# google-deepmind/dm_control

Hardware: AMD Instinct MI355X
Metric: env-steps/s (whole node) at batch 4096; max rel qpos error vs CPU (higher is better)
Workload: dtype f32

## Files before the change

### dm_control_amd/csrc/step_core.h

```cpp
#pragma once
#include <math.h>
#include <stdint.h>
#ifdef DMC_HOST_EMU
#include <stdio.h>
#include <stdlib.h>
#include <string.h>
#endif

#include "../../include/dmc_model_layout.h"
#include "step_layout.h"

#ifdef DMC_HOST_EMU
#define DMC_DEV inline
#define DMC_FN inline
#define DMC_LDS
#define DMC_GLB
#define DMC_WSYNC() ((void)++dmc_emu_wsync_count)
static long long dmc_emu_wsync_count = 0;
#else
#define DMC_DEV __device__ __forceinline__
#define DMC_FN __device__ __attribute__((noinline, not_tail_called))
#define DMC_LDS __attribute__((address_space(3)))
#define DMC_GLB __attribute__((address_space(1)))
#define DMC_WSYNC()                                             \
// ... 2625 lines not shown
      const int a0 = MI(level_adr)[lev], cnt = MI(level_adr)[lev + 1] - a0;
      for (int idx = lane; idx < cnt*6; idx += LPE) {
        const int b = MI(level_body)[a0 + idx/6], comp = idx % 6;
        const int c0 = MI(child_adr)[b], c1 = MI(child_adr)[b + 1];
        if (c1 > c0) {
          T v = S(cfrc)[6*b + comp];
          for (int c = c0; c < c1; c++) v += S(cfrc)[6*MI(child_list)[c] + comp];
          S(cfrc)[6*b + comp] = v;
        }
      }
      DMC_WSYNC();
    }
    FOR_LANES(i, nv) S(qfrc_bias)[i] = dot_n(S(cdof) + 6*i, S(cfrc) + 6*MI(dof_bodyid)[i], 6);
    DMC_WSYNC();
  }

  DMC_DEV void subtree_linvel_sensors() {
    for (int k = 0; k < L.d.nstv; k++) {
      const int sidx = MI(stv_sensor)[k], root = MI(sensor_objid)[sidx];
      T mom[3] = {0, 0, 0};
      FOR_LANES(i, L.d.nbody) {
        const unsigned m = (unsigned)(root < 32 ? MI(body_anc_lo)[i] : MI(body_anc_hi)[i]);
        if (!((m >> (root & 31)) & 1u)) continue;
        const T* rc = S(subtree_com) + 3*MI(body_rootid)[i];
        T dif[3] = {S(xipos)[3*i] - rc[0], S(xipos)[3*i + 1] - rc[1], S(xipos)[3*i + 2] - rc[2]}, tmp[3];
        cross3(tmp, dif, S(cvel) + 6*i);
        for (int c = 0; c < 3; c++) mom[c] += MR(body_mass)[i] * (S(cvel)[6*i + 3 + c] - tmp[c]);
      }
      const T inv = 1 / t_max((T)DMC_MINVAL, MR(body_subtreemass)[root]);
      for (int c = 0; c < 3; c++) { const T v = group_sum<LPE>(mom[c]) * inv; if (lane == 0) S(sensordata)[MI(sensor_adr)[sidx] + c] = v; }
    }
  }
  DMC_DEV void object_velocity(int body, const T* pos, const T* mat, T* res) {
    const T* rc = S(subtree_com) + 3*MI(body_rootid)[body];
    T dif[3] = {pos[0] - rc[0], pos[1] - rc[1], pos[2] - rc[2]}, tmp[3];
    const T* cv = S(cvel) + 6*body;
    cross3(tmp, dif, cv);
    T lin[3] = {cv[3] - tmp[0], cv[4] - tmp[1], cv[5] - tmp[2]};
    mul_matT_vec3(res, mat, cv); mul_matT_vec3(res + 3, mat, lin);
  }
  DMC_DEV void contact_force_local(int c, T* f6) {
    for (int k = 0; k < 6; k++) f6[k] = 0;
    const int r0 = SI(con_efc)[c];
    if (r0 < 0) return;
    const int dim = con_dim(c);
    const T* f = S(efc_force) + r0;
    if (dim == 1) { f6[0] = f[0]; return; }
    if (L.d.elliptic) { for (int k = 0; k < dim; k++) f6[k] = f[k]; return; }
    for (int k = 0; k < 2*(dim - 1); k++) f6[0] += f[k];
    for (int k = 1; k < dim; k++) f6[k] = (f[2*(k - 1)] - f[2*(k - 1) + 1]) * MR(prm_friction)[3*con_prm(c) + (k < 3 ? 0 : (k == 3 ? 1 : 2))];
  }
  DMC_DEV void rne_post_constraint() {
    const int nb = L.d.nbody, ncon = SI(imisc)[IM_NCON];
    FOR_LANES(b, nb) {
      T acc[6] = {0, 0, 0, 0, 0, 0};
      if (b > 0) for (int c = 0; c < ncon; c++) {
        if (SI(con_efc)[c] < 0) continue;
        const int b1 = con_b1(c), b2 = con_b2(c);
        if (b1 != b && b2 != b) continue;
        T lf[6], gf[3], gt[3], dif[3], t[3];
        contact_force_local(c, lf);
        mul_matT_vec3(gf, conF() + 9*c, lf); mul_matT_vec3(gt, conF() + 9*c, lf + 3);
        const T* rc = S(subtree_com) + 3*MI(body_rootid)[b];
        for (int k = 0; k < 3; k++) dif[k] = S(con_pos)[3*c + k] - rc[k];
        cross3(t, dif, gf);
        if (b1 == b) for (int k = 0; k < 3; k++) { acc[k] += -(gt[k] + t[k]); acc[3 + k] += -gf[k]; }
        if (b2 == b) for (int k = 0; k < 3; k++) { acc[k] += (gt[k] + t[k]); acc[3 + k] += gf[k]; }
      }
      if (b > 0 && o.xfrc) {
        T xf[6], dif[3], t[3]; load_xfrc(b, xf);
        const T* rc = S(subtree_com) + 3*MI(body_rootid)[b];
        for (int k = 0; k < 3; k++) dif[k] = S(xipos)[3*b + k] - rc[k];
        cross3(t, dif, xf);
        for (int k = 0; k < 3; k++) { acc[k] += xf[3 + k] + t[k]; acc[3 + k] += xf[k]; }
      }
      for (int k = 0; k < 6; k++) S(cfrc_ext)[6*b + k] = acc[k];
    }
    if (lane == 0) {
      T* ca = S(cacc);
      ca[0] = ca[1] = ca[2] = 0; ca[3] = ca[4] = ca[5] = 0;
      if (!(o.disableflags & DMC_DSBL_GRAVITY)) { ca[3] = -o.gravity[0]; ca[4] = -o.gravity[1]; ca[5] = -o.gravity[2]; }
      for (int k = 0; k < 6; k++) S(cfrc)[k] = 0;
    }
    DMC_WSYNC();
    for (int lev = 0; lev < L.d.nlevel; lev++) {
      const int a0 = MI(level_adr)[lev], a1 = MI(level_adr)[lev + 1];
      for (int kk = a0 + lane; kk < a1; kk += LPE) {
        const int i = MI(level_body)[kk], bda = MI(body_dofadr)[i];
        T csum[6], tmp[6], tmp1[6], tmp2[6];
        for (int a = 0; a < 6; a++) csum[a] = S(cacc)[6*MI(body_parentid)[i] + a];
        for (int k = 0; k < MI(body_dofnum)[i]; k++) for (int a = 0; a < 6; a++)
          csum[a] += SG(cdof_dot)[6*(bda + k) + a]*S(qvel)[bda + k] + S(cdof)[6*(bda + k) + a]*S(qacc)[bda + k];
        for (int a = 0; a < 6; a++) S(cacc)[6*i + a] = csum[a];
        mul_inert_vec(tmp, SG(cinert) + 10*i, csum);
        mul_inert_vec(tmp1, SG(cinert) + 10*i, S(cvel) + 6*i);
        cross_force(tmp2, S(cvel) + 6*i, tmp1);
        for (int a = 0; a < 6; a++) S(cfrc)[6*i + a] = tmp[a] + tmp2[a] - S(cfrc_ext)[6*i + a];
      }
      DMC_WSYNC();
    }
    for (int lev = L.d.nlevel - 2; lev >= 0; lev--) {
      const int a0 = MI(level_adr)[lev], cnt = MI(level_adr)[lev + 1] - a0;
      for (int idx = lane; idx < cnt*6; idx += LPE) {
        const int b = MI(level_body)[a0 + idx/6], comp = idx % 6;
        const int c0 = MI(child_adr)[b], c1 = MI(child_adr)[b + 1];
        if (c1 > c0) {
// ... 1936 lines not shown
          if (lane == 0) S(efc_force)[i] = f;
          if (delta != 0) { const T* Ap = ns_A() + i*cap; for (int b = lane; b < nefc; b += LPE) S(ns_res)[b] += Ap[b]*delta; }
          DMC_WSYNC();
          improvement -= change;
        } else if (dim == 3) improvement -= pgs_cone_block<3>(i);
        else if (dim == 4) improvement -= pgs_cone_block<4>(i);
        else improvement -= pgs_cone_block<6>(i);
        i += dim;
      }
      improvement *= scale;
      iter++;
      if (improvement < o.tolerance) break;
    }
    constraint_force_to_joint(nefc);
    DMC_WSYNC();
    chol_solve(S(sv_Mgrad), M_factor(), S(qfrc_constraint), nv, true);
    FOR_LANES(i, nv) { const T a = S(qacc_smooth)[i] + S(sv_Mgrad)[i]; S(qacc)[i] = a; S(qacc_warmstart)[i] = a; }
    if (lane == 0) SI(imisc)[IM_ITER] = iter;
    DMC_WSYNC();
  }
  DMC_DEV void fwd_constraint() {
    const int nv = L.d.nv, nefc = SI(imisc)[IM_NEFC];
    if (!nefc) {
      FOR_LANES(i, nv) { const T a = S(qacc_smooth)[i]; S(qacc)[i] = a; S(qacc_warmstart)[i] = a; S(qfrc_constraint)[i] = 0; }
      if (lane == 0) SI(imisc)[IM_ITER] = 0;
      DMC_WSYNC();
      return;
    }
    if (L.d.pgs) {
      pgs_solve(nefc);
      if (L.d.nslip) { if (o.noslip_iterations > 0) noslip(nefc); }
      return;
    }
    int changed = 1;
    T cc = 0, gauss = 0;
    bool evaluated = false;
    if (!(o.disableflags & DMC_DSBL_WARMSTART)) {
      jar_from(S(qacc_smooth), nefc);
      DMC_WSYNC();
      const T cs = constraint_update(nefc);
      FOR_LANES(i, nv) S(qacc)[i] = S(qacc_warmstart)[i];
      DMC_WSYNC();
      jar_from(S(qacc), nefc);
      mul_M(S(sv_Ma), S(qacc));
      DMC_WSYNC();
      for (int i = lane; i < nefc; i += LPE) SI(efc_active)[i] = -1;
      cc = constraint_update(nefc, &changed);
      gauss = gauss_cost();
      if (cc + gauss > cs) FOR_LANES(i, nv) S(qacc)[i] = S(qacc_smooth)[i];
      else evaluated = true;
    } else FOR_LANES(i, nv) S(qacc)[i] = S(qacc_smooth)[i];
    DMC_WSYNC();
    int iter;
    if (L.d.island && (o.islands < 0 ? (sizeof(T) == 8 || L.d.cg) : o.islands != 0) && !(o.disableflags & DMC_DSBL_ISLAND) && solve_islands(nefc, &iter)) constraint_force_to_joint(nefc);
    else {
      iter = primal_solve(nefc, evaluated, cc, gauss, changed);
    }
    FOR_LANES(i, nv) S(qacc_warmstart)[i] = S(qacc)[i];
    if (lane == 0) SI(imisc)[IM_ITER] = iter;
    DMC_WSYNC();
    DMC_PROF(PROF_SOL_UPD);
    if (L.d.nslip) { if (o.noslip_iterations > 0) noslip(nefc); }
    DMC_PROF(PROF_NOSLIP);
  }
#if !defined(DMC_HOST_EMU) && !defined(DMC_NO_NEWTON_REGS)
#ifndef DMC_NEWTON_REGS_F64_NV
#define DMC_NEWTON_REGS_F64_NV 0
#endif
  static constexpr bool kNewtonRegs = LS::kNV > 0 && LS::kNV <= 16 && LS::kNV <= LPE && LPE >= 16
                                      && (sizeof(T) == 4 || LS::kNV <= DMC_NEWTON_REGS_F64_NV);
#else
  static constexpr bool kNewtonRegs = false;
#endif
#ifndef DMC_EPS_IMP
#define DMC_EPS_IMP 1
#endif
  static constexpr int kNewtonRows = 16;
#ifndef DMC_HOST_EMU
  template <int N> DMC_DEV T nr_dot(const T (&m)[N], T v) const {
#pragma clang fp contract(off)
    T s = 0;
#pragma unroll
    for (int j = 0; j < N; j++) { const T t = m[j] * bcast_rows<LPE, N>(v, j); s = s + t; }
    return s;
  }
  DMC_DEV T nr_jtf(const T (&Jc)[kNewtonRows], T force, int nefc) const {
#pragma clang fp contract(off)
    T f = 0;
#pragma unroll
    for (int r = 0; r < kNewtonRows; r += 4) if (r < nefc) {
      T fr[4];
#pragma unroll
      for (int u = 0; u < 4; u++) fr[u] = bcast_rows<LPE, kNewtonRows>(force, r + u);
#pragma unroll
      for (int u = 0; u < 4; u++) {
        if constexpr (sizeof(T) == 4) { if (u < 2) { const T t = Jc[r + u]*fr[u]; f = f + t; } else f = __builtin_fmaf(Jc[r + u], fr[u], f); }
        else f = fr[u] != 0 ? f + Jc[r + u]*fr[u] : f;
      }
    }
    return f;
  }
  template <int N> DMC_DEV void nr_factor(const T (&M)[N], const T (&Jc)[kNewtonRows], T wD, int nefc, T (&row)[N], T (&col)[N], T& dinv) const {
    const bool own = lane < N;
    T a[N];
#pragma unroll
    for (int j = 0; j < N; j++) { a[j] = M[j]; col[j] = 0; }
#pragma unroll
    for (int r = 0; r < kNewtonRows; r += 4) if (r < nefc) {
      T c[4];
#pragma unroll
      for (int u = 0; u < 4; u++) c[u] = bcast_rows<LPE, kNewtonRows>(wD, r + u)*Jc[r + u];
#pragma unroll
      for (int u = 0; u < 4; u++) {
#pragma unroll
        for (int j = 0; j < N; j++) a[j] += c[u] * bcast_rows<LPE, N>(Jc[r + u], j);
      }
    }
    dinv = 0;
#pragma unroll
    for (int k = 0; k < N; k++) {
      T akk = bcast_rows<LPE, N>(a[k], k);
      if (akk < (T)DMC_MINVAL) akk = (T)DMC_MINVAL;
      const T inv = t_rsqrt(akk);
      const T lik = a[k] * inv;
#pragma unroll
      for (int j = k + 1; j < N; j++) {
        const T ljk = bcast_rows<LPE, N>(lik, j);
        a[j] = nmsub<true>(a[j], lik, ljk);
        col[j] = lane == k ? ljk : col[j];
      }
      row[k] = (own && k < lane) ? lik : (T)0;
      dinv = lane == k ? inv : dinv;
    }
  }
  template <int N> DMC_DEV T nr_solve(const T (&row)[N], const T (&col)[N], T dinv, T b) const {
    T sreg = lane < N ? b : (T)0;
#pragma unroll
    for (int k = 0; k < N; k++) { const T xk = bcast_rows<LPE, N>(sreg*dinv, k); sreg = nmsub<true>(sreg, row[k], xk); }
    sreg = sreg*dinv;
#pragma unroll
    for (int k = N - 1; k >= 0; k--) { const T xk = bcast_rows<LPE, N>(sreg*dinv, k); sreg = nmsub<true>(sreg, col[k], xk); }
    return sreg*dinv;
  }
  DMC_DEV T nr_update(bool rown, T jar, T D, T& force, int& act, int* changed) const {
    T cost = 0;
    int ch = 0;
    if (rown) {
      const int a = jar < 0;
      const T dj = D*jar;
      force = a ? -dj : (T)0;
      if (sizeof(T) == 4) cost += a ? (T)0.5*dj*jar : (T)0; else if (a) cost += (T)0.5*D*jar*jar;
      ch |= act != a; act = a;
    }
    cost = group_sum<LPE>(cost);
    *changed = group_max<LPE>(ch);
    return cost;
  }
  template <int N>
  DMC_DEV int primal_solve_regs(int nefc, bool evaluated, T cc, T gauss, int changed) {
    const bool own = lane < N, rown = lane < nefc;
    const int i = own ? lane : 0, rl = rown ? lane : 0;
    const T scale = 1 / (o.meaninertia * (T)(N > 1 ? N : 1));
    constexpr bool keep = sizeof(T) == 4;
    T M[N], Jr[N], Jc[kNewtonRows], row[N], col[N], dinv = 0;
    auto load_M = [&]() __attribute__((always_inline)) {
      asm volatile("" ::: "memory");
#pragma unroll
      for (int j = 0; j < N; j++) M[j] = S(qM)[i*N + j];
    };
    auto load_Jr = [&]() __attribute__((always_inline)) {
#pragma unroll
      for (int j = 0; j < N; j++) Jr[j] = S(efc_Jd)[rl*N + j];
    };
    load_M(); load_Jr();
#pragma unroll
    for (int r = 0; r < kNewtonRows; r++) {
      const int t = r & ~3, rr = r < nefc ? r : (t < nefc ? t : 0);
      Jc[r] = S(efc_Jd)[rr*N + i];
    }
    T qacc = S(qacc)[i];
    const T qas = S(qacc_smooth)[i], qfs = S(qfrc_smooth)[i];
    const T D_ = S(efc_D)[rl], aref_ = S(efc_aref)[rl], Ma_ = S(sv_Ma)[i], jar_ = S(efc_jar)[rl], force_ = S(efc_force)[rl];
    const int act_ = SI(efc_active)[rl];
    const T D = rown ? D_ : (T)0;
    T Ma, jar, force = 0;
    int act;
    auto gauss_cost_regs = [&]() __attribute__((always_inline)) {
      T g = 0;
      if (own) g += (Ma - qfs) * (qacc - qas);
      return (T)0.5 * group_sum<LPE>(g);
    };
    if (!evaluated) {
      Ma = nr_dot<N>(M, qacc);
      const T ja = nr_dot<N>(Jr, qacc) - aref_;
      jar = rown ? ja : (T)0;
      changed = 1;
      act = -1;
      cc = nr_update(rown, jar, D, force, act, &changed);
      gauss = gauss_cost_regs();
    } else { Ma = Ma_; jar = rown ? jar_ : (T)0; force = rown ? force_ : (T)0; act = act_; }
    T cost = cc + gauss;
    DMC_PROF(PROF_SOL_INIT);
    T fc, grad, Mgrad;
    auto gradient_regs = [&](int refactor) __attribute__((always_inline)) {
      fc = nr_jtf(Jc, force, nefc);
      grad = Ma - qfs - fc;
      DMC_PROF(PROF_SOL_GRAD);
      if (refactor) {
        if constexpr (!keep) load_M();
        nr_factor<N>(M, Jc, (rown && act == EFC_ST_QUADRATIC) ? D : (T)0, nefc, row, col, dinv);
        DMC_PROF(PROF_FACTOR);
      }
      Mgrad = nr_solve<N>(row, col, dinv, grad);
      DMC_PROF(PROF_SOLVE);
    };
    gradient_regs(1);
    T search = -Mgrad;
    DMC_PROF(PROF_SOL_GRAD);
    int iter = 0;
    const bool anch = anchored();
    while (iter < o.iterations) {
      if (iter == DMC_PRIO_ITER) __builtin_amdgcn_s_setprio(2);
      T lscost = 0;
      DMC_TSUB(3, iter == 0, 4);
      if constexpr (!keep) { load_M(); load_Jr(); }
      const T Mv = nr_dot<N>(M, search);
      const T jv_ = nr_dot<N>(Jr, search);
      const T jv = rown ? jv_ : (T)0;
      T a1 = 0, a2 = 0, a3 = 0, a4 = 0;
      if (own) {
        const T sr = search;
        if (anch) a1 += sr*grad;
        else { a1 += sr*Ma; a2 += qfs*sr; }
        a3 += sr*Mv; a4 += sr*sr;
      }
      LSPre pre;
      pre.a1 = a1; pre.a2 = a2; pre.a3 = a3; pre.a4 = a4; pre.jar = jar; pre.jv = jv; pre.D = D;
      const T alpha = primal_search<true>(nefc, gauss, scale, &lscost, pre);
      DMC_PROF(PROF_SOL_LS);
      DMC_TSUB(3, iter == 0, 5);
      if (alpha == 0) break;
      if constexpr (sizeof(T) == 4) {
        qacc = __builtin_fmaf(alpha, search, qacc); Ma = __builtin_fmaf(alpha, Mv, Ma);
        jar = __builtin_fmaf(alpha, jv, jar);
      } else { qacc += alpha*search; Ma += alpha*Mv; jar += alpha*jv; }
      const T oldcost = cost;
      cc = nr_update(rown, jar, D, force, act, &changed);
      gauss = gauss_cost_regs();
      cost = cc + gauss;
      DMC_PROF(PROF_SOL_UPD);
      DMC_TSUB(3, iter == 0, 6);
      gradient_regs(changed);
      DMC_PROF(PROF_SOL_GRAD);
      DMC_TSUB(3, iter == 0, 7);
      T g2 = 0, ma2 = 0;
      search = -Mgrad;
      if (own) { g2 += grad*grad; ma2 += Ma*Ma; }
      g2 = group_sum<LPE>(g2); ma2 = group_sum<LPE>(ma2);
      const T improvement = ls_relative<T>() ? -scale*lscost : scale*(oldcost - cost), gradient = scale*t_sqrt(g2);
      iter++;
      const T ulp = sizeof(T) == 4 ? (T)1.1920929e-7 : (T)2.220446049250313e-16;
      const T tol_imp = ls_relative<T>() ? o.tolerance : t_max(o.tolerance, (T)DMC_EPS_IMP*ulp*scale*t_abs(cost));
      const bool exact_step = sizeof(T) == 4 && !changed && t_abs(alpha - 1) < (T)1e-3;
      const T tol_grad = t_max(o.tolerance, (exact_step ? 64 : 8)*ulp*scale*t_sqrt(ma2));
      if (improvement < tol_imp || gradient < tol_grad) break;
    }
    __builtin_amdgcn_s_setprio(0);
    if (own) { S(qacc)[lane] = qacc; S(qfrc_constraint)[lane] = fc; }
    if (rown) { S(efc_force)[lane] = force; S(efc_jar)[lane] = jar; SI(efc_active)[lane] = act; }
    DMC_WSYNC();
    return iter;
  }
#endif
  DMC_DEV int primal_solve(int nefc, bool evaluated, T cc, T gauss, int changed) {
#ifndef DMC_HOST_EMU
    if constexpr (kNewtonRegs) {
      if (L.d.jfull && !L.d.msparse && !L.d.elliptic && !L.d.cg && !L.d.nslip && !general_rows() && nefc <= kNewtonRows)
        return primal_solve_regs<LS::kNV>(nefc, evaluated, cc, gauss, changed);
    }
#endif
    const int nv = L.d.nv;
    const T scale = 1 / (o.meaninertia * (T)(nv > 1 ? nv : 1));
    if (!evaluated) {
      mul_M(S(sv_Ma), S(qacc));
      jar_from(S(qacc), nefc);
      DMC_WSYNC();
      changed = 1;
      for (int i = lane; i < nefc; i += LPE) SI(efc_active)[i] = -1;
      cc = constraint_update(nefc, &changed);
      gauss = gauss_cost();
    }
    T cost = cc + gauss;
#ifdef DMC_HOST_EMU
    hsplit = !L.d.cg && h_split(nefc);
    emu_split_solves() += hsplit ? 1 : 0;
#else
    hsplit = false;
    if constexpr (kSplit) hsplit = !L.d.cg && h_split(nefc);
#endif
#ifdef DMC_HOST_EMU
    if (getenv("DMC_EMU_TRACE_SPLIT")) fprintf(stderr, "h_split %d (treemax %d, ncon %d)\n", (int)hsplit, L.d.treemax, SI(imisc)[IM_NCON]);
#endif
    DMC_PROF(PROF_SOL_INIT);
    newton_gradient(nefc, 1);
    FOR_LANES(i, nv) S(sv_search)[i] = -S(sv_Mgrad)[i];
    DMC_WSYNC();
    DMC_PROF(PROF_SOL_GRAD);
    int iter = 0, stall = 0;
    T gbest = (T)DMC_MAXVAL;
#ifndef DMC_STALL_ITERS
#define DMC_STALL_ITERS 6
#endif
    while (iter < o.iterations) {
#ifndef DMC_HOST_EMU
      if (iter == DMC_PRIO_ITER) __builtin_amdgcn_s_setprio(2);
#endif
      T lscost;
      DMC_TSUB(3, iter == 0, 4);
      const T alpha = primal_search(nefc, gauss, scale, &lscost);
      DMC_PROF(PROF_SOL_LS);
      DMC_TSUB(3, iter == 0, 5);
#ifdef DMC_HOST_EMU
      if (getenv("DMC_EMU_TRACE_LS")) fprintf(stderr, "    ls returned alpha %.9e lscost %.6e\n", (double)alpha, (double)lscost);
#endif
      if (alpha == 0) break;
      FOR_LANES(i, nv) { S(qacc)[i] += alpha*S(sv_search)[i]; S(sv_Ma)[i] += alpha*S(sv_Mv)[i]; }
// ... 117 lines not shown
      const u64 C = isl_comp(t);
      if (!C || ctz64(C) != t || !(C & rowtrees)) continue;
      FOR_LANES(i, nv) S(qacc)[i] = ((C >> dof_root(i)) & 1) ? S(qacc_warmstart)[i] : S(qacc_smooth)[i];
      for (int r = lane; r < nefc; r += LPE) if (!(row_trees(r) & C)) S(efc_D)[r] *= eps;
      DMC_WSYNC();
      const int it = primal_solve(nefc, false, 0, 0, 1);
      FOR_LANES(i, nv) if ((C >> dof_root(i)) & 1) S(qacc_warmstart)[i] = S(qacc)[i];
      for (int r = lane; r < nefc; r += LPE) if (!(row_trees(r) & C)) S(efc_D)[r] *= 1 / eps;
      DMC_WSYNC();
      if (it > itmax) itmax = it;
    }
    FOR_LANES(i, nv) S(qacc)[i] = ((covered >> dof_root(i)) & 1) ? S(qacc_warmstart)[i] : S(qacc_smooth)[i];
    DMC_WSYNC();
    jar_from(S(qacc), nefc);
    DMC_WSYNC();
    constraint_update(nefc);
    DMC_WSYNC();
    *iter_out = itmax;
    return true;
  }

  DMC_DEV void euler_state() {
    const int nv = L.d.nv;
    const T dt = o.timestep;
    const T* qacc = S(qacc);
    const bool implicitfast = kFeat && o.integrator == DMC_INT_IMPLICITFAST;
    if (implicitfast) {
      FOR_LANES(i, nv) {
        T dd = (o.disableflags & DMC_DSBL_DAMPER) ? (T)0 : MR(dof_damping)[i];
        if (!(o.disableflags & DMC_DSBL_ACTUATION)) for (int a = 0; a < L.d.nu; a++) {
          const int fl = MI(act_flags)[a];
          if ((fl & ACTF_TENDON) || MI(act_dof)[a] != i) continue;
          if (fl & ACTF_FORCELIMITED) { const T f = S(actuator_force)[a]; if (f <= MRC(act_forcerange)[2*a] || f >= MRC(act_forcerange)[2*a + 1]) continue; }
          T bv = (fl & ACTF_BIAS_AFFINE) ? MRC(act_biasprm)[3*a + 2] : (T)0;
          const T gv = (fl & ACTF_GAIN_AFFINE) ? MRC(act_gainprm)[3*a + 2] : (T)0;
          if (gv != 0) bv += gv * ((L.d.na && (fl & ACTF_DYN_ANY)) ? S(act)[MI(act_adr)[a]] : S(ctrl)[a]);
          const T gear = MRC(act_gear)[a];
          dd -= gear*gear*bv;
        }
        S(sv_search)[i] = dd;
      }
      DMC_WSYNC();
    }
    if (L.d.na) FOR_LANES(i, L.d.nu) {
      const int fl = MI(act_flags)[i];
      if (fl & ACTF_DYN_ANY) {
        const int k = MI(act_adr)[i];
        if (fl & ACTF_DYN_FILTEREXACT) { const T tau = t_max((T)DMC_MINVAL, MR(act_dynprm)[i]); S(act)[k] += S(act_dot)[k] * tau * (1 - t_exp(-dt/tau)); }
        else S(act)[k] += dt*S(act_dot)[k];
        if (fl & ACTF_ACTLIMITED) S(act)[k] = t_max(MRC(act_actrange)[2*i], t_min(MRC(act_actrange)[2*i + 1], S(act)[k]));
      }
    }
    if (implicitfast || (o.any_damping && !(o.disableflags & (DMC_DSBL_EULERDAMP | DMC_DSBL_DAMPER)))) {
      FOR_LANES(i, nv) S(sv_grad)[i] = S(qfrc_smooth)[i] + S(qfrc_constraint)[i];
      DMC_WSYNC();
      factor_M(true, implicitfast ? S(sv_search) : MR(dof_damping));
      chol_solve(S(sv_Mgrad), S(qLH), S(sv_grad), nv, true);
      qacc = S(sv_Mgrad);
    }
    FOR_LANES(i, nv) S(qvel)[i] += dt*qacc[i];
    DMC_WSYNC();
    FOR_LANES(j, L.d.njnt) {
      const int qa = MI(jnt_qposadr)[j], da = MI(jnt_dofadr)[j], t = MI(jnt_type)[j];
      if (t == DMC_JNT_FREE) {
        for (int k = 0; k < 3; k++) S(qpos)[qa + k] += dt*S(qvel)[da + k];
        T q[4], w[3];
        for (int k = 0; k < 4; k++) q[k] = S(qpos)[qa + 3 + k];
        for (int k = 0; k < 3; k++) w[k] = S(qvel)[da + 3 + k];
        quat_integrate(q, w, dt);
        for (int k = 0; k < 4; k++) S(qpos)[qa + 3 + k] = q[k];
      } else if (t == DMC_JNT_BALL) {
        T q[4], w[3];
        for (int k = 0; k < 4; k++) q[k] = S(qpos)[qa + k];
        for (int k = 0; k < 3; k++) w[k] = S(qvel)[da + k];
        quat_integrate(q, w, dt);
        for (int k = 0; k < 4; k++) S(qpos)[qa + k] = q[k];
      } else S(qpos)[qa] += dt*S(qvel)[da];
    }
    DMC_WSYNC();
  }
  DMC_DEV void euler() { euler_state(); time_ += o.timestep_d; }

  DMC_DEV void integrate_pos_from(const T* q0, const T* vel, T h) {
    FOR_LANES(j, L.d.njnt) {
      const int qa = MI(jnt_qposadr)[j], da = MI(jnt_dofadr)[j], t = MI(jnt_type)[j];
      if (t == DMC_JNT_FREE || t == DMC_JNT_BALL) {
        int qo = qa, dofo = da;
        if (t == DMC_JNT_FREE) { for (int k = 0; k < 3; k++) S(qpos)[qa + k] = q0[qa + k] + h*vel[da + k]; qo += 3; dofo += 3; }
        T q[4], w[3];
        for (int k = 0; k < 4; k++) q[k] = q0[qo + k];
        for (int k = 0; k < 3; k++) w[k] = vel[dofo + k];
        quat_integrate(q, w, h);
        for (int k = 0; k < 4; k++) S(qpos)[qo + k] = q[k];
      } else S(qpos)[qa] = q0[qa] + h*vel[da];
    }
  }
  DMC_DEV void rk4_stage(int stage) {
    const int nv = L.d.nv;
    const T h = o.timestep;
    const T Bw = (stage == 0 || stage == 3) ? (T)(1.0/6) : (T)(1.0/3);
    if (stage == 0) {
      FOR_LANES(i, L.d.nq) S(rk_q0)[i] = S(qpos)[i];
      FOR_LANES(i, nv) { S(rk_v0)[i] = S(qvel)[i]; S(rk_dq)[i] = Bw*S(qvel)[i]; S(rk_dv)[i] = Bw*S(qacc)[i]; }
    } else FOR_LANES(i, nv) { S(rk_dq)[i] += Bw*S(qvel)[i]; S(rk_dv)[i] += Bw*S(qacc)[i]; }
    DMC_WSYNC();
    if (stage < 3) {
      const T a = stage == 2 ? (T)1 : (T)0.5;
      FOR_LANES(i, nv) { S(sv_grad)[i] = a*S(qvel)[i]; S(sv_Mgrad)[i] = a*S(qacc)[i]; }
      DMC_WSYNC();
      integrate_pos_from(S(rk_q0), S(sv_grad), h);
      FOR_LANES(i, nv) S(qvel)[i] = S(rk_v0)[i] + h*S(sv_Mgrad)[i];
      DMC_WSYNC();
    }
  }
  DMC_DEV void rk4_finish() {
    const T h = o.timestep;
    FOR_LANES(i, L.d.nv) S(qvel)[i] = S(rk_v0)[i] + h*S(rk_dv)[i];
    integrate_pos_from(S(rk_q0), S(rk_dq), h);
    time_ += o.timestep_d;
    DMC_WSYNC();
  }

  DMC_DEV void reset_state() {
    FOR_LANES(i, L.d.nq) S(qpos)[i] = MR(qpos0)[i];
    FOR_LANES(i, L.d.nv) { S(qvel)[i] = 0; S(qacc_warmstart)[i] = 0; S(qfrc_applied)[i] = 0; }
    FOR_LANES(i, L.d.nu) S(ctrl)[i] = 0;
    if (L.d.na) FOR_LANES(i, L.d.na) { S(act)[i] = 0; S(act_dot)[i] = 0; }
    time_ = 0;
    DMC_WSYNC();
  }
  DMC_DEV bool check_pos_vel() {
    int badp = 0, badv = 0;
    FOR_LANES(i, L.d.nq) if (t_bad(S(qpos)[i])) badp = 1;
    badp = group_max<LPE>(badp);
    if (badp) { if (lane == 0) SI(imisc)[IM_WARN + DMC_WARN_BADQPOS]++; if (!(o.disableflags & DMC_DSBL_AUTORESET)) { DMC_WSYNC(); reset_state(); } }
    FOR_LANES(i, L.d.nv) if (t_bad(S(qvel)[i])) badv = 1;
    badv = group_max<LPE>(badv);
    if (badv) { if (lane == 0) SI(imisc)[IM_WARN + DMC_WARN_BADQVEL]++; if (!(o.disableflags & DMC_DSBL_AUTORESET)) { DMC_WSYNC(); reset_state(); } }
    return (badp || badv) && !(o.disableflags & DMC_DSBL_AUTORESET);
  }
  DMC_DEV bool bad_acc() {
    int bad = 0;
    FOR_LANES(i, L.d.nv) if (t_bad(S(qacc)[i])) bad = 1;
    return group_max<LPE>(bad) != 0;
  }

  DMC_DEV void stage_posvel(bool partial, int outmask, bool skipsensor, bool havekin = false) {
    if (!havekin) { kinematics(); DMC_PROF(PROF_KIN); DMC_TSUB(1, partial, 4); com_pos(); DMC_PROF(PROF_COM); DMC_TSUB(1, partial, 5); }
    if (!partial) { crb_mass_matrix(); DMC_PROF(PROF_CRB); DMC_TSUB(2, true, 4); }
    if (!partial || (outmask & (OUT_CONTACT | OUT_CONTACT_IDS))) { collision(); DMC_PROF(PROF_COLL); DMC_TSUB(2, !partial, 5); }
    if (!partial) { make_constraint(); DMC_PROF(PROF_CONSTR); DMC_TSUB(2, true, 6); }
    if (!skipsensor) sensors(DMC_STAGE_POS);
    DMC_PROF(PROF_SENS);
    DMC_TSUB(1, partial, 6);
    if (!havekin) { com_vel(); DMC_PROF(PROF_COMVEL); DMC_TSUB(1, partial, 7); }
    if (!partial) { passive_and_rne(); DMC_PROF(PROF_RNE); DMC_TSUB(2, true, 7); }
    if (!skipsensor) sensors(DMC_STAGE_VEL);
    DMC_PROF(PROF_SENS);
  }
  DMC_DEV void stage_acc(bool disable_actuation, bool skipsensor) {
    fwd_actuation(disable_actuation); DMC_PROF(PROF_ACT); fwd_acceleration(); DMC_PROF(PROF_ACC); fwd_constraint();
    DMC_PROF(PROF_X8);
    if (!skipsensor) sensors_acc();
    DMC_PROF(PROF_SENS);
  }
  DMC_DEV void sub_stamp(int row) {
#if defined(DMC_TRACE_SUB) && !defined(DMC_HOST_EMU)
    const StepIO<T>* iop = (const StepIO<T>*)((const unsigned char*)&o + (sizeof(StepOpts<T>) + 15) / 16 * 16);
    if (iop->trace && (threadIdx.x & 63) == 0) {
      const int epw = 64 / LPE, nitems = (iop->B + epw - 1) / epw;
      iop->trace[((size_t)(iop->trace_slot & 7) * 8 + row) * nitems + SI(imisc)[IM_ENV] / epw] = (int)(wall_clock64() & 0x7fffffffll);
    }
#else
    (void)row;
#endif
  }
  DMC_DEV void trace_stamp(const StepIO<T>& io, int env, int row) {
#if !defined(DMC_HOST_EMU) && !defined(DMC_TRACE_SUB)
    if (io.trace && (threadIdx.x & 63) == 0) {
      const int epw = 64 / LPE, nitems = (io.B + epw - 1) / epw;
      io.trace[((size_t)(io.trace_slot & 7) * 8 + row) * nitems + env / epw] = (int)(wall_clock64() & 0x7fffffffll);
    }
#else
    (void)io; (void)env; (void)row;
#endif
  }
  DMC_DEV void prof_begin() {
#if defined(DMC_PROFILE) && !defined(DMC_HOST_EMU)
    if (lane == 0) { for (int k = 0; k < 33; k++) SI(prof)[k] = 0; SI(prof)[33] = (int)__builtin_readcyclecounter(); }
#endif
  }
  DMC_DEV void prof_end(const StepIO<T>& io, int env) {
#if defined(DMC_PROFILE) && !defined(DMC_HOST_EMU)
    if (io.prof && lane == 0) for (int k = 0; k < 32; k++) io.prof[(size_t)k*io.B + env] += SI(prof)[k];
#else
    (void)io; (void)env;
#endif
  }
#ifndef DMC_HOST_EMU
  DMC_DEV void call_posvel(bool partial, int outmask, bool skipsensor, bool havekin = false) {
    StageFns<T, LPE, LS>::posvel(ls, (const DMC_LDS StepOpts<T>*)&o, (DMC_LDS int*)mi, (DMC_LDS T*)mr, gc, (DMC_LDS T*)s,
                                 (DMC_LDS int*)si, lane, (partial ? 1 : 0) | (skipsensor ? 2 : 0) | (havekin ? 4 : 0), outmask);
  }
  DMC_DEV void call_acc(bool disable_actuation, bool skipsensor) {
    StageFns<T, LPE, LS>::acc(ls, (const DMC_LDS StepOpts<T>*)&o, (DMC_LDS int*)mi, (DMC_LDS T*)mr, gc, (DMC_LDS T*)s,
                              (DMC_LDS int*)si, lane, (disable_actuation ? 1 : 0) | (skipsensor ? 2 : 0));
  }
  DMC_DEV void call_euler() {
    StageFns<T, LPE, LS>::euler(ls, (const DMC_LDS StepOpts<T>*)&o, (DMC_LDS int*)mi, (DMC_LDS T*)mr, gc, (DMC_LDS T*)s,
                                (DMC_LDS int*)si, lane);
    time_ += o.timestep_d;
  }
#else
  DMC_DEV void call_posvel(bool partial, int outmask, bool skipsensor, bool havekin = false) { stage_posvel(partial, outmask, skipsensor, havekin); }
  DMC_DEV void call_acc(bool disable_actuation, bool skipsensor) { stage_acc(disable_actuation, skipsensor); }
  DMC_DEV void call_euler() { euler(); }
#endif
  DMC_DEV void load_ctrl_seq(const StepIO<T>& io, int env, int t) {
    env = late(env);
    const int B = io.B, nu = L.d.nu;
    DMC_WSYNC();
    FOR_LANES(i, nu) S(ctrl)[i] = io.ctrl_seq[((size_t)t*nu + i)*B + env];
    DMC_WSYNC();
  }
  DMC_DEV void store_seq(const StepIO<T>& io, int env, int t) {
    env = late(env);
    const int B = io.B;
    if (io.qpos_seq) FOR_LANES(i, L.d.nq) io.qpos_seq[((size_t)t*L.d.nq + i)*B + env] = S(qpos)[i];
    if (io.qvel_seq) FOR_LANES(i, L.d.nv) io.qvel_seq[((size_t)t*L.d.nv + i)*B + env] = S(qvel)[i];
    if (io.sensor_seq) FOR_LANES(i, L.d.nsensordata) io.sensor_seq[((size_t)t*L.d.nsensordata + i)*B + env] = S(sensordata)[i];
  }
  DMC_DEV void run_split(const StepIO<T>& io, int env, int mode, int outmask, const Entry& en) {
    const bool stash = io.stash_r != nullptr;
    bool have = false;
    if (lane == 0) set_epoch(en.epoch);
    DMC_WSYNC();
    if (mode == 5 && stash) have = load_stash(io, env);
    load_state(io, env, have, en);
    if (mode == 4) {
      check_pos_vel();
      call_posvel(false, outmask, false);
      store_outputs(io, env, outmask);
      if (stash) store_stash(io, env, true);
      store_state(io, env);
      return;
    }
    int retried = 0;
    for (;;) {
      if (!have || retried) call_posvel(false, outmask, true);
      call_acc(false, false);
      if (!retried && bad_acc()) {
        if (lane == 0) SI(imisc)[IM_WARN + DMC_WARN_BADQACC]++;
        if (!(o.disableflags & DMC_DSBL_AUTORESET)) { DMC_WSYNC(); reset_state(); retried = 1; continue; }
      }
      break;
    }
    store_outputs(io, env, outmask & (OUT_SENSOR | OUT_QACC | OUT_ACTUATOR | OUT_QFRC | OUT_CONTACT));
    call_euler();
    if (stash) store_stash(io, env, false);
    store_state(io, env);
  }
  DMC_DEV TaskLds<T> task_lds() const {
    TaskLds<T> v;
    v.qpos = S(qpos); v.qvel = S(qvel); v.ctrl = S(ctrl); v.act = S(act); v.sensordata = S(sensordata); v.xpos = S(xpos);
    v.xmat = S(xmat); v.xipos = S(xipos); v.subtree_com = S(subtree_com); v.geom_xpos = S(geom_xpos); v.cvel = S(cvel);
    return v;
  }
  DMC_DEV void probe_store(const StepIO<T>& io, int env, int first, int count) {
    if constexpr (!kFeat) return;
    env = late(env);
    T* p = io.probe;
    if (!p) return;
    const int cap = io.probe_cap, g = io.probe_geom;
    for (int t = first; t < first + count && t < cap; t++) FOR_LANES(k, 3) p[((size_t)t*3 + k)*io.B + env] = S(geom_xpos)[3*g + k];
  }
  DMC_DEV void run(const StepIO<T>& io, int env, int nstep, int legacy, int mode, int outmask, int nsub) {
    Entry en; EntryRegs er;
    entry_issue(L, o, io, env, lane, mode, legacy, &en, &er);
    entry_commit(L, io, env, lane, &en, er, s);
    run(io, env, nstep, legacy, mode, outmask, nsub, en);
  }
  DMC_DEV void run(const StepIO<T>& io, int env, int nstep, int legacy, int mode, int outmask, int nsub, const Entry& en,
                   int piece = 0, int npieces = 1) {
    const int launch_mode = mode;
    if (lane == 0) set_epoch(en.epoch);
    if (io.env_mode) {
      const int em = en.em;
      if (em == 2) return;
      if (em == 1 && (mode == 0 || mode >= 4)) mode = 2;
    }
    if constexpr (!kSlices) { piece = 0; npieces = 1; }
    if (mode != 0 && piece != npieces - 1) return;
    if (mode != 0) { piece = 0; npieces = 1; }
    if (mode >= 4) { run_split(io, env, mode, outmask, en); return; }
    prof_begin();
    const bool stash = io.stash_r != nullptr;
    bool have = false;
    if (stash && mode == 0 && legacy && o.integrator != DMC_INT_RK4) have = load_stash(io, env);
    load_state(io, env, have, en, kSlices && piece > 0);
    bool havekin = false;
    if (piece == 0 && io.kstash && mode == 0 && launch_mode == 0 && legacy && !have && o.integrator != DMC_INT_RK4) {
      if (!en.fast) havekin = load_kstash(io, env);
      else if (en.kvalid) { havekin = true; DMC_WSYNC(); kstash_env_geoms(); }
    }
    DMC_PROF(PROF_LOAD);
    const bool stepping = mode == 0 || mode == 3;
    const int ntotal = mode == 3 ? nstep*nsub : nstep;
    const int npass = !stepping ? 1 : ntotal + ((legacy || mode == 3) ? 1 : 0);
    const bool fwd_after = kFeat && legacy == 2 && mode == 0;
    const bool last_piece = piece == npieces - 1;
    const int it_lo = npieces > 1 ? (int)((long long)piece * ntotal / npieces) : 0;
    const int it_hi = (npieces > 1 && !last_piece) ? (int)((long long)(piece + 1) * ntotal / npieces) : npass;
    for (int it = it_lo; it < it_hi; it++) {
      const bool trailing = stepping && it == ntotal;
      const bool partial = trailing && !(stash && mode == 0) && !fwd_after;
      if (mode == 3 && !trailing && it % nsub == 0 && io.ctrl_seq) load_ctrl_seq(io, env, it / nsub);
      if (stepping) { if (check_pos_vel()) { have = false; havekin = false; } }
      const int nstage = (stepping && !trailing && o.integrator == DMC_INT_RK4) ? 4 : 1;
      const bool sens_pv = !stepping || it == npass - 1 || (mode == 3 && it % nsub == 0);
      const bool sens_acc = !stepping || (it == ntotal - 1 && !fwd_after) || (trailing && fwd_after) || (mode == 3 && (it + 1) % nsub == 0);
      int stage = 0, retried = 0;
      while (stage < nstage) {
        if (!(have && it == 0 && !retried)) call_posvel(partial, outmask, stage > 0 || !sens_pv, havekin && it == 0 && !retried && !trailing);
        if (it == 0 && stage == 0) trace_stamp(io, env, 4); else if (trailing) trace_stamp(io, env, 7);
        if (mode == 3 && stage == 0 && it > 0 && it % nsub == 0) store_seq(io, env, it / nsub - 1);
        if (mode == 0 && stage == 0 && it >= 1) probe_store(io, env, it - 1, 1);
        if (trailing && !fwd_after) break;
        call_acc(mode == 2, stage > 0 || !sens_acc);
        if (trailing) break;
        if (it == 0 && stage == 0) trace_stamp(io, env, 5);
        if (stage == 0 && stepping && !retried && bad_acc()) {
          if (lane == 0) SI(imisc)[IM_WARN + DMC_WARN_BADQACC]++;
          if (!(o.disableflags & DMC_DSBL_AUTORESET)) { DMC_WSYNC(); reset_state(); retried = 1; continue; }
        }
        if (stage == 0 && stepping && it == ntotal - 1) { dump_debug(io, env); if (mode == 0 && !legacy) store_outputs(io, env, outmask); }
        if (nstage > 1) rk4_stage(stage);
        stage++;
      }
      if (!stepping || trailing) break;
      if (nstage > 1) rk4_finish(); else call_euler();
      if (it == 0) trace_stamp(io, env, 6);
      DMC_PROF(PROF_EULER);
    }
    if constexpr (kSlices) if (!last_piece) { store_handoff(io, env); DMC_PROF(PROF_STORE); prof_end(io, env); return; }
    if (!stepping) dump_debug(io, env);
    if (!stepping && launch_mode == 0) probe_store(io, env, 0, nstep);
    if (!stepping || legacy || mode == 3) { DMC_PROF(PROF_TRAIL); store_outputs(io, env, outmask); }
    if (stash) store_stash(io, env, mode == 0 && legacy && !fwd_after);
    if (io.kstash && mode == 0 && legacy && o.integrator != DMC_INT_RK4) store_kstash(io, env);
    store_state(io, env);
    DMC_PROF(PROF_STORE);
    prof_end(io, env);
  }
#undef MI
#undef MR
#undef GC
#undef S
#undef SG
#undef SI
#undef FOR_LANES
};


#ifndef DMC_HOST_EMU
template <typename T, int LPE, typename LS>
struct StageFns {
  typedef StepCore<T, LPE, LS> Core;
  static DMC_FN void posvel(LS ls, const DMC_LDS StepOpts<T>* o, DMC_LDS int* mi, DMC_LDS T* mr, const int* gc, DMC_LDS T* s,
                            DMC_LDS int* si, int lane, int flags, int outmask) {
    Core c(ls, *(const StepOpts<T>*)o, (const int*)mi, (const T*)mr, gc, (T*)s, (int*)si, lane);
    c.stage_posvel(flags & 1, outmask, flags & 2, flags & 4);
  }
  static DMC_FN void acc(LS ls, const DMC_LDS StepOpts<T>* o, DMC_LDS int* mi, DMC_LDS T* mr, const int* gc, DMC_LDS T* s,
                         DMC_LDS int* si, int lane, int flags) {
    Core c(ls, *(const StepOpts<T>*)o, (const int*)mi, (const T*)mr, gc, (T*)s, (int*)si, lane);
    c.stage_acc(flags & 1, flags & 2);
  }
  static DMC_FN void ns_build(LS ls, const DMC_LDS StepOpts<T>* o, DMC_LDS int* mi, DMC_LDS T* mr, const int* gc, DMC_LDS T* s,
                              DMC_LDS int* si, int lane, int nf) {
    if constexpr (LS::kNV > 0 && LS::kNV <= 32 && LPE == 64) {
      Core c(ls, *(const StepOpts<T>*)o, (const int*)mi, (const T*)mr, gc, (T*)s, (int*)si, lane);
      c.template noslip_build_A_lanes<LS::kNV>((const DMC_LDS T*)c.M_factor(), nf, c.row_map());
    }
  }
  static DMC_FN void euler(LS ls, const DMC_LDS StepOpts<T>* o, DMC_LDS int* mi, DMC_LDS T* mr, const int* gc, DMC_LDS T* s,
                           DMC_LDS int* si, int lane) {
    Core c(ls, *(const StepOpts<T>*)o, (const int*)mi, (const T*)mr, gc, (T*)s, (int*)si, lane);
    c.euler_state();
  }
};
#endif

}
```

Baseline: 76.55 million.

## Fuse smooth acceleration, constraint solve and damped Euler solve into register path

For small dense models with few constraint rows, stage_acc now runs a register-resident path that computes qfrc_smooth/qacc_smooth from the existing M factor, does the warmstart comparison and Newton solve in registers, and skips fwd_acceleration/fwd_constraint. When a plain Euler step with damping follows, it also factors M+dt*damping in registers and solves for the next qacc, and flags euler() to skip its own factor and solve. This removes LDS round trips and wave syncs between stages. It adds register pressure and a shared flag in misc, and the result may differ numerically from the LDS path.

```diff
diff --git a/dm_control_amd/csrc/step_core.h b/dm_control_amd/csrc/step_core.h
--- a/dm_control_amd/csrc/step_core.h
+++ b/dm_control_amd/csrc/step_core.h
@@ -2701,6 +2701,7 @@
   }
   DMC_DEV void rne_post_constraint() {
     const int nb = L.d.nbody, ncon = SI(imisc)[IM_NCON];
+    if constexpr (kAccRegs) { if (lane == 0) S(misc)[kMiscEulerSolved] = 0; }
     FOR_LANES(b, nb) {
       T acc[6] = {0, 0, 0, 0, 0, 0};
       if (b > 0) for (int c = 0; c < ncon; c++) {
@@ -4743,7 +4744,7 @@
     } else FOR_LANES(i, nv) S(qacc)[i] = S(qacc_smooth)[i];
     DMC_WSYNC();
     int iter;
-    if (L.d.island && (o.islands < 0 ? (sizeof(T) == 8 || L.d.cg) : o.islands != 0) && !(o.disableflags & DMC_DSBL_ISLAND) && solve_islands(nefc, &iter)) constraint_force_to_joint(nefc);
+    if (islands_on() && solve_islands(nefc, &iter)) constraint_force_to_joint(nefc);
     else {
       iter = primal_solve(nefc, evaluated, cc, gauss, changed);
     }
@@ -4767,6 +4768,12 @@
 #define DMC_EPS_IMP 1
 #endif
   static constexpr int kNewtonRows = 16;
+#if !defined(DMC_NO_ACC_REGS)
+  static constexpr bool kAccRegs = kNewtonRegs;
+#else
+  static constexpr bool kAccRegs = false;
+#endif
+  static constexpr int kMiscEulerSolved = 2;
 #ifndef DMC_HOST_EMU
   template <int N> DMC_DEV T nr_dot(const T (&m)[N], T v) const {
 #pragma clang fp contract(off)
@@ -4844,11 +4851,39 @@
       ch |= act != a; act = a;
     }
     cost = group_sum<LPE>(cost);
-    *changed = group_max<LPE>(ch);
+    if (changed) *changed = group_max<LPE>(ch);
     return cost;
   }
-  template <int N>
-  DMC_DEV int primal_solve_regs(int nefc, bool evaluated, T cc, T gauss, int changed) {
+  template <int N> DMC_DEV void nr_factor_diag(const T (&M)[N], T dt, T d, T (&row)[N], T (&col)[N], T& dinv) const {
+#pragma clang fp contract(off)
+    const bool own = lane < N;
+    const T dv = dt*d;
+    T a[N];
+#pragma unroll
+    for (int j = 0; j < N; j++) {
+      T v = M[j] + dv;
+      if constexpr (sizeof(T) == 4) { if (j == N - 1 && (N & 1)) v = __builtin_fmaf(dt, d, M[j]); }
+      a[j] = (j == lane) ? v : M[j]; col[j] = 0;
+    }
+    dinv = 0;
+#pragma unroll
+    for (int k = 0; k < N; k++) {
+      T akk = bcast_rows<LPE, N>(a[k], k);
+      if (akk < (T)DMC_MINVAL) akk = (T)DMC_MINVAL;
+      const T inv = t_rsqrt(akk);
+      const T lik = a[k] * inv;
+#pragma unroll
+      for (int j = k + 1; j < N; j++) {
+        const T ljk = bcast_rows<LPE, N>(lik, j);
+        a[j] = nmsub<true>(a[j], lik, ljk);
+        col[j] = lane == k ? ljk : col[j];
+      }
+      row[k] = (own && k < lane) ? lik : (T)0;
+      dinv = lane == k ? inv : dinv;
+    }
+  }
+  template <int N, bool ACC = false>
+  DMC_DEV int primal_solve_regs(int nefc, bool evaluated, T cc, T gauss, int changed, bool euler_next = false) {
     const bool own = lane < N, rown = lane < nefc;
     const int i = own ? lane : 0, rl = rown ? lane : 0;
     const T scale = 1 / (o.meaninertia * (T)(N > 1 ? N : 1));
@@ -4869,10 +4904,29 @@
       const int t = r & ~3, rr = r < nefc ? r : (t < nefc ? t : 0);
       Jc[r] = S(efc_Jd)[rr*N + i];
     }
-    T qacc = S(qacc)[i];
-    const T qas = S(qacc_smooth)[i], qfs = S(qfrc_smooth)[i];
-    const T D_ = S(efc_D)[rl], aref_ = S(efc_aref)[rl], Ma_ = S(sv_Ma)[i], jar_ = S(efc_jar)[rl], force_ = S(efc_force)[rl];
-    const int act_ = SI(efc_active)[rl];
+    T qacc, qas, qfs, Ma_ = 0, jar_ = 0, force_ = 0;
+    int act_ = 0;
+    const T D_ = S(efc_D)[rl], aref_ = S(efc_aref)[rl];
+    if constexpr (ACC) {
+      const DMC_LDS T* Lm = (const DMC_LDS T*)M_factor();
+      const int ci = tri_c0(i, N);
+      T mrow[N], mcol[N];
+#pragma unroll
+      for (int k = 0; k < N; k++) {
+        const T r_ = Lm[tri_c0(k, N) + ((own && k < i) ? i - k : 0)], c_ = Lm[ci + ((own && k > i) ? k - i : 0)];
+        mrow[k] = (own && k < i) ? r_ : (T)0; mcol[k] = (own && k > i) ? c_ : (T)0;
+      }
+      const T mdinv_ = Lm[ci];
+      const T fp = S(qfrc_passive)[i], fb = S(qfrc_bias)[i], fa = S(qfrc_applied)[i], fu = S(qfrc_actuator)[i];
+      qacc = S(qacc_warmstart)[i];
+      qfs = fp - fb + fa + fu;
+      qas = nr_solve<N>(mrow, mcol, own ? mdinv_ : (T)0, qfs);
+      if (own) { S(qfrc_smooth)[lane] = qfs; S(qacc_smooth)[lane] = qas; }
+      DMC_PROF(PROF_ACC);
+    } else {
+      qacc = S(qacc)[i]; qas = S(qacc_smooth)[i]; qfs = S(qfrc_smooth)[i];
+      Ma_ = S(sv_Ma)[i]; jar_ = S(efc_jar)[rl]; force_ = S(efc_force)[rl]; act_ = SI(efc_active)[rl];
+    }
     const T D = rown ? D_ : (T)0;
     T Ma, jar, force = 0;
     int act;
@@ -4881,7 +4935,7 @@
       if (own) g += (Ma - qfs) * (qacc - qas);
       return (T)0.5 * group_sum<LPE>(g);
     };
-    if (!evaluated) {
+    auto evaluate = [&]() __attribute__((always_inline)) {
       Ma = nr_dot<N>(M, qacc);
       const T ja = nr_dot<N>(Jr, qacc) - aref_;
       jar = rown ? ja : (T)0;
@@ -4889,10 +4943,26 @@
       act = -1;
       cc = nr_update(rown, jar, D, force, act, &changed);
       gauss = gauss_cost_regs();
-    } else { Ma = Ma_; jar = rown ? jar_ : (T)0; force = rown ? force_ : (T)0; act = act_; }
+    };
+    T fc = 0, grad = 0, Mgrad = 0;
+    int iter = 0;
+    if constexpr (ACC) {
+      if (nefc == 0) qacc = qas;
+      else if (!(o.disableflags & DMC_DSBL_WARMSTART)) {
+        const T js = nr_dot<N>(Jr, qas) - aref_;
+        T f0 = 0;
+        int a0 = 0;
+        const T cs = nr_update(rown, rown ? js : (T)0, D, f0, a0, nullptr);
+        evaluate();
+        if (cc + gauss > cs) { qacc = qas; evaluate(); }
+      } else { qacc = qas; evaluate(); }
+    } else {
+      if (!evaluated) evaluate();
+      else { Ma = Ma_; jar = rown ? jar_ : (T)0; force = rown ? force_ : (T)0; act = act_; }
+    }
+    const bool solve = !ACC || nefc > 0;
     T cost = cc + gauss;
     DMC_PROF(PROF_SOL_INIT);
-    T fc, grad, Mgrad;
     auto gradient_regs = [&](int refactor) __attribute__((always_inline)) {
       fc = nr_jtf(Jc, force, nefc);
       grad = Ma - qfs - fc;
@@ -4905,12 +4975,11 @@
       Mgrad = nr_solve<N>(row, col, dinv, grad);
       DMC_PROF(PROF_SOLVE);
     };
-    gradient_regs(1);
+    if (solve) gradient_regs(1);
     T search = -Mgrad;
     DMC_PROF(PROF_SOL_GRAD);
-    int iter = 0;
     const bool anch = anchored();
-    while (iter < o.iterations) {
+    while (solve && iter < o.iterations) {
       if (iter == DMC_PRIO_ITER) __builtin_amdgcn_s_setprio(2);
       T lscost = 0;
       DMC_TSUB(3, iter == 0, 4);
@@ -4957,12 +5026,31 @@
       if (improvement < tol_imp || gradient < tol_grad) break;
     }
     __builtin_amdgcn_s_setprio(0);
+    if constexpr (ACC) {
+      if (euler_next) {
+        T erow[N], ecol[N], edinv;
+        if constexpr (!keep) load_M();
+        nr_factor_diag<N>(M, o.timestep, MR(dof_damping)[i], erow, ecol, edinv);
+        const T qe = nr_solve<N>(erow, ecol, edinv, qfs + fc);
+        if (own) S(sv_Mgrad)[lane] = qe;
+        if (lane == 0) S(misc)[kMiscEulerSolved] = (T)1;
+      }
+      if (own) S(qacc_warmstart)[lane] = qacc;
+      if (lane == 0) SI(imisc)[IM_ITER] = iter;
+    }
     if (own) { S(qacc)[lane] = qacc; S(qfrc_constraint)[lane] = fc; }
     if (rown) { S(efc_force)[lane] = force; S(efc_jar)[lane] = jar; SI(efc_active)[lane] = act; }
     DMC_WSYNC();
     return iter;
   }
-#endif
+  DMC_DEV bool acc_regs_ok(int nefc) const {
+    return L.d.jfull && !L.d.msparse && !L.d.elliptic && !L.d.cg && !L.d.nslip && !general_rows() && nefc <= kNewtonRows
+           && !L.d.pgs && !o.xfrc && !islands_on();
+  }
+#endif
+  DMC_DEV bool islands_on() const {
+    return L.d.island && (o.islands < 0 ? (sizeof(T) == 8 || L.d.cg) : o.islands != 0) && !(o.disableflags & DMC_DSBL_ISLAND);
+  }
   DMC_DEV int primal_solve(int nefc, bool evaluated, T cc, T gauss, int changed) {
 #ifndef DMC_HOST_EMU
     if constexpr (kNewtonRegs) {
@@ -5186,10 +5274,14 @@
       }
     }
     if (implicitfast || (o.any_damping && !(o.disableflags & (DMC_DSBL_EULERDAMP | DMC_DSBL_DAMPER)))) {
-      FOR_LANES(i, nv) S(sv_grad)[i] = S(qfrc_smooth)[i] + S(qfrc_constraint)[i];
-      DMC_WSYNC();
-      factor_M(true, implicitfast ? S(sv_search) : MR(dof_damping));
-      chol_solve(S(sv_Mgrad), S(qLH), S(sv_grad), nv, true);
+      bool solved = false;
+      if constexpr (kAccRegs) { solved = S(misc)[kMiscEulerSolved] != 0; if (lane == 0) S(misc)[kMiscEulerSolved] = 0; }
+      if (!solved) {
+        FOR_LANES(i, nv) S(sv_grad)[i] = S(qfrc_smooth)[i] + S(qfrc_constraint)[i];
+        DMC_WSYNC();
+        factor_M(true, implicitfast ? S(sv_search) : MR(dof_damping));
+        chol_solve(S(sv_Mgrad), S(qLH), S(sv_grad), nv, true);
+      }
       qacc = S(sv_Mgrad);
     }
     FOR_LANES(i, nv) S(qvel)[i] += dt*qacc[i];
@@ -5260,6 +5352,7 @@
     FOR_LANES(i, L.d.nv) { S(qvel)[i] = 0; S(qacc_warmstart)[i] = 0; S(qfrc_applied)[i] = 0; }
     FOR_LANES(i, L.d.nu) S(ctrl)[i] = 0;
     if (L.d.na) FOR_LANES(i, L.d.na) { S(act)[i] = 0; S(act_dot)[i] = 0; }
+    if constexpr (kAccRegs) { if (lane == 0) S(misc)[kMiscEulerSolved] = 0; }
     time_ = 0;
     DMC_WSYNC();
   }
@@ -5292,8 +5385,22 @@
     if (!skipsensor) sensors(DMC_STAGE_VEL);
     DMC_PROF(PROF_SENS);
   }
-  DMC_DEV void stage_acc(bool disable_actuation, bool skipsensor) {
-    fwd_actuation(disable_actuation); DMC_PROF(PROF_ACT); fwd_acceleration(); DMC_PROF(PROF_ACC); fwd_constraint();
+  DMC_DEV void stage_acc(bool disable_actuation, bool skipsensor, bool euler_next = false) {
+    fwd_actuation(disable_actuation); DMC_PROF(PROF_ACT);
+    bool regs = false;
+#ifndef DMC_HOST_EMU
+    if constexpr (kAccRegs) {
+      const int nefc = SI(imisc)[IM_NEFC];
+      if (lane == 0) S(misc)[kMiscEulerSolved] = 0;
+      regs = acc_regs_ok(nefc);
+      if (regs) {
+        const bool damped = euler_next && o.any_damping && !(o.disableflags & (DMC_DSBL_EULERDAMP | DMC_DSBL_DAMPER))
+                            && !(kFeat && o.integrator == DMC_INT_IMPLICITFAST);
+        primal_solve_regs<LS::kNV, true>(nefc, false, 0, 0, 1, damped);
+      }
+    }
+#endif
+    if (!regs) { fwd_acceleration(); DMC_PROF(PROF_ACC); fwd_constraint(); }
     DMC_PROF(PROF_X8);
     if (!skipsensor) sensors_acc();
     DMC_PROF(PROF_SENS);
@@ -5336,9 +5443,11 @@
     StageFns<T, LPE, LS>::posvel(ls, (const DMC_LDS StepOpts<T>*)&o, (DMC_LDS int*)mi, (DMC_LDS T*)mr, gc, (DMC_LDS T*)s,
                                  (DMC_LDS int*)si, lane, (partial ? 1 : 0) | (skipsensor ? 2 : 0) | (havekin ? 4 : 0), outmask);
   }
-  DMC_DEV void call_acc(bool disable_actuation, bool skipsensor) {
+  DMC_DEV void call_acc(bool disable_actuation, bool skipsensor, bool euler_next = false) {
+    int flags = (disable_actuation ? 1 : 0) | (skipsensor ? 2 : 0);
+    if constexpr (kAccRegs) flags |= euler_next ? 4 : 0;
     StageFns<T, LPE, LS>::acc(ls, (const DMC_LDS StepOpts<T>*)&o, (DMC_LDS int*)mi, (DMC_LDS T*)mr, gc, (DMC_LDS T*)s,
-                              (DMC_LDS int*)si, lane, (disable_actuation ? 1 : 0) | (skipsensor ? 2 : 0));
+                              (DMC_LDS int*)si, lane, flags);
   }
   DMC_DEV void call_euler() {
     StageFns<T, LPE, LS>::euler(ls, (const DMC_LDS StepOpts<T>*)&o, (DMC_LDS int*)mi, (DMC_LDS T*)mr, gc, (DMC_LDS T*)s,
@@ -5347,7 +5456,7 @@
   }
 #else
   DMC_DEV void call_posvel(bool partial, int outmask, bool skipsensor, bool havekin = false) { stage_posvel(partial, outmask, skipsensor, havekin); }
-  DMC_DEV void call_acc(bool disable_actuation, bool skipsensor) { stage_acc(disable_actuation, skipsensor); }
+  DMC_DEV void call_acc(bool disable_actuation, bool skipsensor, bool euler_next = false) { stage_acc(disable_actuation, skipsensor, euler_next); }
   DMC_DEV void call_euler() { euler(); }
 #endif
   DMC_DEV void load_ctrl_seq(const StepIO<T>& io, int env, int t) {
@@ -5382,7 +5491,7 @@
     int retried = 0;
     for (;;) {
       if (!have || retried) call_posvel(false, outmask, true);
-      call_acc(false, false);
+      call_acc(false, false, true);
       if (!retried && bad_acc()) {
         if (lane == 0) SI(imisc)[IM_WARN + DMC_WARN_BADQACC]++;
         if (!(o.disableflags & DMC_DSBL_AUTORESET)) { DMC_WSYNC(); reset_state(); retried = 1; continue; }
@@ -5460,7 +5569,7 @@
         if (mode == 3 && stage == 0 && it > 0 && it % nsub == 0) store_seq(io, env, it / nsub - 1);
         if (mode == 0 && stage == 0 && it >= 1) probe_store(io, env, it - 1, 1);
         if (trailing && !fwd_after) break;
-        call_acc(mode == 2, stage > 0 || !sens_acc);
+        call_acc(mode == 2, stage > 0 || !sens_acc, stepping && !trailing && nstage == 1);
         if (trailing) break;
         if (it == 0 && stage == 0) trace_stamp(io, env, 5);
         if (stage == 0 && stepping && !retried && bad_acc()) {
@@ -5508,7 +5617,7 @@
   static DMC_FN void acc(LS ls, const DMC_LDS StepOpts<T>* o, DMC_LDS int* mi, DMC_LDS T* mr, const int* gc, DMC_LDS T* s,
                          DMC_LDS int* si, int lane, int flags) {
     Core c(ls, *(const StepOpts<T>*)o, (const int*)mi, (const T*)mr, gc, (T*)s, (int*)si, lane);
-    c.stage_acc(flags & 1, flags & 2);
+    c.stage_acc(flags & 1, flags & 2, flags & 4);
   }
   static DMC_FN void ns_build(LS ls, const DMC_LDS StepOpts<T>* o, DMC_LDS int* mi, DMC_LDS T* mr, const int* gc, DMC_LDS T* s,
                               DMC_LDS int* si, int lane, int nf) {
```

Result: faster. 78.34 million, median of 6 (+2.3%).
